# jayleicn/ClipBERT

Hardware: NVIDIA H100
Metric: clips/sec fwd+bwd MSRVTT ret (ResNet50+BERT-base) (higher is better)
Workload: dtype bf16

## Files before the change

### clipbert_b200/csrc/gemm.cu

```cuda
#include "common.cuh"
#include "host_util.h"

namespace cb {

constexpr int BM = 128;
constexpr int BK = 64;
constexpr int CONSUMER_WARPS = 8;
constexpr int GEMM_THREADS = (CONSUMER_WARPS + 1) * 32;
constexpr int PP_THREADS = 3 * 128;
constexpr int PP_PRODUCER_REGS = 40;
constexpr int PP_CONSUMER_REGS = 232;
constexpr int PP_BAR_TURN = 1;
constexpr int MAX_STAGES = 8;
constexpr int SMEM_LIMIT = 232448;
constexpr int SMEM_LIMIT_OCC2 = 113 * 1024;
constexpr int STG_PITCH = 36;
constexpr int STG_WARP_FLOATS = 16 * STG_PITCH;
constexpr int EPI_BYTES = CONSUMER_WARPS * STG_WARP_FLOATS * 4;
constexpr int IN_BOX_BYTES = BM * 64 * 2;

struct GemmEpi {
  const float* scale;
  const float* shift;
  const __nv_bfloat16* residual;
  const __nv_bfloat16* aux;
  int aux_mode;
  int act;
  void* out;
  int64_t out_ld;
  int out_fp32;
  __nv_bfloat16* out2;
  int64_t out2_ld;
  int rowmap, H, W;
  uint32_t drop_thresh;
  float drop_inv_keep;
  uint64_t seed;
  const uint64_t* seed_off;
  int mn3d;
  long long* dbg;
};

__device__ __forceinline__ void dbg_stamp(const GemmEpi& epi, int slot) {
  if (epi.dbg) {
    epi.dbg[blockIdx.x * 32 + slot] = clock64();
    if (slot == 0 || slot == 11) {
      unsigned long long ns;
      asm volatile("mov.u64 %0, %%globaltimer;" : "=l"(ns));
      epi.dbg[blockIdx.x * 32 + (slot == 0 ? 12 : 13)] = static_cast<long long>(ns);
    }
  }
}

template <int BN>
struct GemmCfg {
  static constexpr int A_BYTES = BM * BK * 2;
  static constexpr int B_BYTES = BN * BK * 2;
  static constexpr int STAGE_BYTES = A_BYTES + B_BYTES;
  static constexpr int BAR_BYTES = 256;
};

enum { EK_GENERIC = 0, EK_SHIFT_ACT = 1, EK_RELU_MASK = 2, EK_DROP_RES = 3, EK_GELU_STASH = 4, EK_AUX_MUL = 5 };

template <int NC>
__device__ __forceinline__ void add_shift(float (&f)[NC], const float (&shv)[NC]) {
#pragma unroll
  for (int j = 0; j < NC; ++j) f[j] += shv[j];
}
template <int NC>
__device__ __forceinline__ void add_residual(float (&f)[NC], const uint32_t (&res16)[NC / 2]) {
#pragma unroll
  for (int j = 0; j < NC / 2; ++j) {
    const float2 r2 = unpack_bf16x2(res16[j]);
    f[2 * j] += r2.x;
    f[2 * j + 1] += r2.y;
  }
}
template <int NC>
__device__ __forceinline__ void epilogue_shift_act(float (&f)[NC], const float (&shv)[NC], bool has_shift, const uint32_t (&res16)[NC / 2], bool has_res,
                                                   bool relu) {
  if (has_shift) add_shift<NC>(f, shv);
  if (has_res) add_residual<NC>(f, res16);
  if (relu) {
#pragma unroll
    for (int j = 0; j < NC; ++j) f[j] = fmaxf(f[j], 0.0f);
  }
}
template <int NC>
__device__ __forceinline__ void epilogue_relu_mask(float (&f)[NC], const uint32_t (&res16)[NC / 2], bool has_res, const uint32_t (&aux16)[NC / 2]) {
  if (has_res) add_residual<NC>(f, res16);
#pragma unroll
  for (int j = 0; j < NC / 2; ++j) {
    const uint32_t a = aux16[j];
    f[2 * j] = ((a & 0x8000u) == 0u && (a & 0x7fffu) != 0u) ? f[2 * j] : 0.0f;
    f[2 * j + 1] = ((a & 0x80000000u) == 0u && (a & 0x7fff0000u) != 0u) ? f[2 * j + 1] : 0.0f;
  }
}
template <int NC>
__device__ __forceinline__ void epilogue_drop_res(float (&f)[NC], const float (&shv)[NC], bool has_shift, const uint32_t (&res16)[NC / 2], bool has_res,
                                                  uint64_t dseed, uint64_t didx, uint32_t thresh, float inv_keep) {
  if (has_shift) add_shift<NC>(f, shv);
#pragma unroll
  for (int j = 0; j < NC; j += 4) {
    float m[4];
    dropout_mult4(dseed, didx + j, thresh, inv_keep, m);
    f[j] *= m[0]; f[j + 1] *= m[1]; f[j + 2] *= m[2]; f[j + 3] *= m[3];
  }
  if (has_res) add_residual<NC>(f, res16);
}
template <int NC>
__device__ __forceinline__ void epilogue_gelu_stash(float (&f)[NC], const float (&shv)[NC], bool has_shift, uint32_t (&o2_16)[NC / 2]) {
  if (has_shift) add_shift<NC>(f, shv);
#pragma unroll
  for (int j = 0; j < NC / 2; ++j) {
    float y0, g0, y1, g1;
    gelu_erf_and_grad(f[2 * j], y0, g0);
    gelu_erf_and_grad(f[2 * j + 1], y1, g1);
    f[2 * j] = y0;
    f[2 * j + 1] = y1;
    o2_16[j] = pack_bf16x2(g0, g1);
  }
}
template <int NC>
__device__ __forceinline__ void epilogue_aux_mul(float (&f)[NC], const uint32_t (&res16)[NC / 2], bool has_res, const uint32_t (&aux16)[NC / 2]) {
  if (has_res) add_residual<NC>(f, res16);
#pragma unroll
  for (int j = 0; j < NC / 2; ++j) {
    const float2 a2 = unpack_bf16x2(aux16[j]);
    f[2 * j] *= a2.x;
    f[2 * j + 1] *= a2.y;
  }
}
template <int NC, bool GUARD>
__device__ __forceinline__ void epilogue_math(float (&f)[NC], const GemmEpi& epi, const float (&shv)[NC], bool has_shift, uint64_t dseed, int nb, int N,
                                              int64_t orow, const uint32_t (&res16)[NC / 2], bool has_res, const uint32_t (&aux16)[NC / 2], bool has_aux,
                                              uint32_t (&o2_16)[NC / 2], bool has_out2) {
  if (GUARD && nb >= N) return;
  if (epi.scale) {
#pragma unroll
    for (int j = 0; j < NC; j += 4) {
      if (!GUARD || nb + j + 4 <= N) {
        const float4 s4 = __ldg(reinterpret_cast<const float4*>(epi.scale + nb + j));
        f[j] *= s4.x; f[j + 1] *= s4.y; f[j + 2] *= s4.z; f[j + 3] *= s4.w;
      }
    }
  }
  if (has_shift) add_shift<NC>(f, shv);
  if (epi.drop_thresh) {
    const uint64_t base = static_cast<uint64_t>(orow) * static_cast<uint64_t>(N) + nb;
#pragma unroll
    for (int j = 0; j < NC; j += 4) {
      float m[4];
      dropout_mult4(dseed, base + j, epi.drop_thresh, epi.drop_inv_keep, m);
      f[j] *= m[0]; f[j + 1] *= m[1]; f[j + 2] *= m[2]; f[j + 3] *= m[3];
    }
  }
  if (has_res) add_residual<NC>(f, res16);
  if (epi.act == CB_ACT_GELU_STASH_GRAD) {
#pragma unroll
    for (int j = 0; j < NC / 2; ++j) {
      float y0, g0, y1, g1;
      gelu_erf_and_grad(f[2 * j], y0, g0);
      gelu_erf_and_grad(f[2 * j + 1], y1, g1);
      f[2 * j] = y0;
      f[2 * j + 1] = y1;
      if (has_out2) o2_16[j] = pack_bf16x2(g0, g1);
    }
  } else if (has_out2) {
#pragma unroll
// ... 323 lines not shown
    while (s >= STAGES) { s -= STAGES; ph ^= 1; }
  };
  if (wg == 1) ring_skip(tile_stages);

  const int er = lane & 15, eh = lane >> 4;
  float* stg = reinterpret_cast<float*>(stg_base) + (warp - 4) * STG_WARP_FLOATS;
  const bool has_out2 = epi.out2 != nullptr;
  const bool has_shift = epi.shift != nullptr;
  const bool full = (N & 15) == 0 && epi.scale == nullptr;
  const bool drop = epi.drop_thresh != 0;
  int kind = EK_GENERIC;
  if (full) {
    if (!drop && !has_out2 && !has_aux && (epi.act == CB_ACT_NONE || epi.act == CB_ACT_RELU)) kind = EK_SHIFT_ACT;
    else if (!drop && !has_out2 && !has_shift && has_aux && epi.aux_mode == CB_AUX_RELU_MASK && epi.act == CB_ACT_NONE) kind = EK_RELU_MASK;
    else if (drop && !has_out2 && !has_aux && epi.act == CB_ACT_NONE) kind = EK_DROP_RES;
    else if (!drop && has_out2 && !has_aux && !has_res && epi.act == CB_ACT_GELU_STASH_GRAD) kind = EK_GELU_STASH;
    else if (!drop && !has_out2 && !has_shift && has_aux && epi.aux_mode == CB_AUX_MUL && epi.act == CB_ACT_NONE) kind = EK_AUX_MUL;
  }
  const bool kind_relu = epi.act == CB_ACT_RELU;
  const bool guard = (N & 15) != 0;

  for (int local = wg, tile = unit + wg * n_units; tile < total_tiles; local += 2, tile += 2 * n_units) {
    const TileInfo t = decode_tile<BN, MODE>(tile, tiles_m, tiles_n, K, ntaps, 0);
    if (local > 0) named_bar_sync(PP_BAR_TURN + wg, 2 * 128);
    const int pass = tile + n_units < total_tiles ? PP_BAR_TURN + (wg ^ 1) : 0;
    mma_tile_pp<BN, MODE != 0>(acc, smem0, stage_bytes, KCH, STAGES, n_iters, lane, s, ph, full_bar, empty_bar, pass, in_stage);

    const uint32_t in_buf = N_IN ? smem_u32(in_base) + (N_IN == 2 ? wg : 0) * in_bytes : smem0 + s * stage_bytes;
    if (in_bytes) {
      if (N_IN) mbar_wait_unguarded(&in_full[wg], static_cast<uint32_t>(local >> 1) & 1u);
      else mbar_wait_unguarded(&full_bar[s], ph);
    }
    int orow_half[2];
#pragma unroll
    for (int h = 0; h < 2; ++h) {
      const int m = t.m0 + h * 64 + wq * 16 + er;
      bool row_ok = m < M;
      int64_t orow = m;
      if (epi.rowmap == CB_ROWMAP_PAD) {
        const int hw = epi.H * epi.W;
        const int img = m / hw;
        const int r = m - img * hw;
        const int y = r / epi.W, x = r - y * epi.W;
        orow = (static_cast<int64_t>(img) * (epi.H + 2) + y + 1) * (epi.W + 2) + x + 1;
      } else if (epi.rowmap == CB_ROWMAP_UNPAD) {
        const int wp = epi.W + 2, hp = epi.H + 2;
        const int img = m / (hp * wp);
        const int r = m - img * (hp * wp);
        const int y = r / wp, x = r - y * wp;
        row_ok = row_ok && y >= 1 && y <= epi.H && x >= 1 && x <= epi.W;
        orow = (static_cast<int64_t>(img) * epi.H + (y - 1)) * epi.W + (x - 1);
      }
      orow_half[h] = row_ok ? static_cast<int>(orow) : -1;
    }
#pragma unroll
    for (int sc = 0; sc < BN / 32; ++sc) {
#pragma unroll 1
      for (int h = 0; h < 2; ++h) {
        const int wrow = h * 64 + wq * 16;
        __syncwarp();
#pragma unroll
        for (int jj = 0; jj < 4; ++jj) {
          const int j = sc * 4 + jj;
          float* p = stg + (lane >> 2) * STG_PITCH + jj * 8 + 2 * (lane & 3);
          const bool h1 = h != 0;
          *reinterpret_cast<float2*>(p) = make_float2(h1 ? acc[1][4 * j] : acc[0][4 * j], h1 ? acc[1][4 * j + 1] : acc[0][4 * j + 1]);
          *reinterpret_cast<float2*>(p + 8 * STG_PITCH) =
              make_float2(h1 ? acc[1][4 * j + 2] : acc[0][4 * j + 2], h1 ? acc[1][4 * j + 3] : acc[0][4 * j + 3]);
        }
        __syncwarp();
        const int nb = t.n0 + sc * 32 + eh * 16;
        const int64_t orow = h ? orow_half[1] : orow_half[0];
        if (orow < 0 || nb >= N) continue;
        constexpr int NC = 16;
        float f[NC];
        const uint32_t srow = smem_u32(stg + er * STG_PITCH + eh * 16);
#pragma unroll
        for (int j = 0; j < NC / 4; ++j) {
          const uint4 u = lds128(srow + j * 16);
          f[4 * j] = __uint_as_float(u.x); f[4 * j + 1] = __uint_as_float(u.y);
          f[4 * j + 2] = __uint_as_float(u.z); f[4 * j + 3] = __uint_as_float(u.w);
        }
        uint32_t res16[NC / 2], aux16[NC / 2];
        const int tc = sc * 32 + eh * 16;
        const int q = (tc & 63) >> 3;
        if (has_res) {
#pragma unroll
          for (int j = 0; j < 2; ++j) {
            const uint4 u = lds128(swz128(in_buf + (tc >> 6) * IN_BOX_BYTES, wrow + er, q + j));
            res16[4 * j] = u.x; res16[4 * j + 1] = u.y; res16[4 * j + 2] = u.z; res16[4 * j + 3] = u.w;
          }
        }
        if (has_aux) {
#pragma unroll
          for (int j = 0; j < 2; ++j) {
            const uint4 u = lds128(swz128(in_buf + (has_res ? IN_TILE_BYTES : 0) + (tc >> 6) * IN_BOX_BYTES, wrow + er, q + j));
            aux16[4 * j] = u.x; aux16[4 * j + 1] = u.y; aux16[4 * j + 2] = u.z; aux16[4 * j + 3] = u.w;
          }
        }
        float shv[NC];
        if (has_shift) {
#pragma unroll
          for (int j = 0; j < NC; j += 4) {
            float4 s4 = make_float4(0.f, 0.f, 0.f, 0.f);
            if (nb + j + 4 <= N) s4 = __ldg(reinterpret_cast<const float4*>(epi.shift + nb + j));
            shv[j] = s4.x; shv[j + 1] = s4.y; shv[j + 2] = s4.z; shv[j + 3] = s4.w;
          }
        }
        uint32_t o2_16[NC / 2];
        switch (kind) {
          case EK_SHIFT_ACT: epilogue_shift_act<NC>(f, shv, has_shift, res16, has_res, kind_relu); break;
          case EK_RELU_MASK: epilogue_relu_mask<NC>(f, res16, has_res, aux16); break;
          case EK_DROP_RES:
            epilogue_drop_res<NC>(f, shv, has_shift, res16, has_res, dseed, static_cast<uint64_t>(orow) * static_cast<uint64_t>(N) + nb,
                                  epi.drop_thresh, epi.drop_inv_keep);
            break;
          case EK_GELU_STASH: epilogue_gelu_stash<NC>(f, shv, has_shift, o2_16); break;
          case EK_AUX_MUL: epilogue_aux_mul<NC>(f, res16, has_res, aux16); break;
          default:
            if (guard) epilogue_math<NC, true>(f, epi, shv, has_shift, dseed, nb, N, orow, res16, has_res, aux16, has_aux, o2_16, has_out2);
            else epilogue_math<NC, false>(f, epi, shv, has_shift, dseed, nb, N, orow, res16, has_res, aux16, has_aux, o2_16, has_out2);
        }
        if (epi.out_fp32) {
          float* o = reinterpret_cast<float*>(epi.out) + orow * epi.out_ld + nb;
#pragma unroll
          for (int j = 0; j < NC; j += 4)
            if (nb + j + 4 <= N) *reinterpret_cast<float4*>(o + j) = make_float4(f[j], f[j + 1], f[j + 2], f[j + 3]);
        } else {
          __nv_bfloat16* o = reinterpret_cast<__nv_bfloat16*>(epi.out) + orow * epi.out_ld + nb;
#pragma unroll
          for (int j = 0; j < 2; ++j)
            if (nb + 8 * j + 8 <= N)
              *reinterpret_cast<uint4*>(o + 8 * j) = make_uint4(pack_bf16x2(f[8 * j], f[8 * j + 1]), pack_bf16x2(f[8 * j + 2], f[8 * j + 3]),
                                                                pack_bf16x2(f[8 * j + 4], f[8 * j + 5]), pack_bf16x2(f[8 * j + 6], f[8 * j + 7]));
        }
        if (has_out2) {
          __nv_bfloat16* o = epi.out2 + orow * epi.out2_ld + nb;
#pragma unroll
          for (int j = 0; j < 2; ++j)
            if (nb + 8 * j + 8 <= N) *reinterpret_cast<uint4*>(o + 8 * j) = make_uint4(o2_16[4 * j], o2_16[4 * j + 1], o2_16[4 * j + 2], o2_16[4 * j + 3]);
        }
      }
    }
    if (in_bytes) {
      __syncwarp();
      if (lane == 0) mbar_arrive(N_IN ? &in_empty[N_IN == 2 ? wg : 0] : &empty_bar[s]);
      if (!N_IN && ++s == STAGES) { s = 0; ph ^= 1; }
    }
    ring_skip(tile_stages);
  }
  if (threadIdx.x == 4 * 32) dbg_stamp(epi, 11);
}

template <int BN, int OCC>
__global__ void __launch_bounds__(GEMM_THREADS, OCC)
    gemm_kernel(const __grid_constant__ CUtensorMap tmA, const __grid_constant__ CUtensorMap tmB, int M, int N, int K, int ntaps, int tap_w,
                int tap_sign, int iters_per_split, int tiles_m, int tiles_n, int total_tiles, int STAGES, int KCH, GemmEpi epi) {
  using Cfg = GemmCfg<BN>;
  extern __shared__ uint8_t smem_raw[];
  uint8_t* smem = reinterpret_cast<uint8_t*>((reinterpret_cast<uintptr_t>(smem_raw) + 1023) & ~static_cast<uintptr_t>(1023));
  const int stage_bytes = KCH * Cfg::STAGE_BYTES;
  uint64_t* full_bar = reinterpret_cast<uint64_t*>(smem + STAGES * stage_bytes);
  uint64_t* empty_bar = full_bar + MAX_STAGES;

  const int warp = threadIdx.x >> 5;
  const int lane = threadIdx.x & 31;
  const int unit = blockIdx.x;
  const int n_units = gridDim.x;
  if (threadIdx.x == 0) dbg_stamp(epi, 0);
  pdl_trigger();
  if (threadIdx.x == 0) {
    tma_prefetch_desc(&tmA);
    tma_prefetch_desc(&tmB);
    for (int s = 0; s < STAGES; ++s) {
      mbar_init(&full_bar[s], 1);
      mbar_init(&empty_bar[s], CONSUMER_WARPS);
    }
    fence_mbar_init();
  }
  __syncthreads();
  pdl_wait();
  if (threadIdx.x == 0) dbg_stamp(epi, 1);

  if (warp >= CONSUMER_WARPS) {
    if (warp == CONSUMER_WARPS && lane == 0) {
      int s = 0;
      uint32_t ph = 0;
      for (int tile = unit; tile < total_tiles; tile += n_units) {
        const TileInfo t = decode_tile<BN, 1>(tile, tiles_m, tiles_n, K, ntaps, iters_per_split);
        int shift = 0;
        if (ntaps == 9) shift = tap_sign * ((t.tap / 3 - 1) * tap_w + (t.tap % 3 - 1));
        for (int i = 0; i < t.n_iters; i += KCH) {
          const int nch = min(KCH, t.n_iters - i);
          mbar_wait(&empty_bar[s], ph ^ 1);
          mbar_expect_tx(&full_bar[s], nch * Cfg::STAGE_BYTES);
          int kit = t.it_begin + i;
          for (int ch = 0; ch < nch; ++ch, ++kit) {
            uint8_t* sa = smem + s * stage_bytes + ch * Cfg::STAGE_BYTES;
            uint8_t* sb = sa + Cfg::A_BYTES;
            const int p = kit * BK;
            if (epi.mn3d) {
              tma_load_3d(sa, &tmA, &full_bar[s], 0, p, t.m0 >> 6);
              tma_load_3d(sb, &tmB, &full_bar[s], 0, p + shift, t.nb0 >> 6);
            } else {
#pragma unroll
              for (int j = 0; j < BM / 64; ++j) tma_load_2d(sa + j * (BK * 128), &tmA, &full_bar[s], t.m0 + j * 64, p);
#pragma unroll
              for (int j = 0; j < BN / 64; ++j) tma_load_2d(sb + j * (BK * 128), &tmB, &full_bar[s], t.nb0 + j * 64, p + shift);
            }
          }
          if (++s == STAGES) { s = 0; ph ^= 1; }
          if (i == 0 && tile == unit) dbg_stamp(epi, 2);
        }
      }
      dbg_stamp(epi, 3);
    }
    return;
  }

  const int wg = warp >> 2;
  const int wrow = wg * 64 + (warp & 3) * 16;
  const uint32_t smem0 = smem_u32(smem);
  float acc[BN / 2];
  int s = 0;
  uint32_t ph = 0;
  int local = 0;
  for (int tile = unit; tile < total_tiles; tile += n_units, ++local) {
    const TileInfo t = decode_tile<BN, 1>(tile, tiles_m, tiles_n, K, ntaps, iters_per_split);
    if (local == 0 && warp == 0 && lane == 0) dbg_stamp(epi, 4);
    mma_tile<BN, 1, 1>(acc, smem0, stage_bytes, KCH, STAGES, t.n_iters, wg, lane, s, ph, full_bar, empty_bar);
    if (local == 0 && warp == 0 && lane == 0) dbg_stamp(epi, 5);
    wgrad_epilogue<BN>(acc, reinterpret_cast<float*>(epi.out) + static_cast<int64_t>(t.tap) * N, epi.out_ld, epi.scale, M, N,
                       t.m0 + wrow + (lane >> 2), t.n0, lane);
    if (local == 0 && warp == 0 && lane == 0) dbg_stamp(epi, 8);
  }
  if (threadIdx.x == 0) dbg_stamp(epi, 11);
}

static int g_sm_limit = 0;
static int sm_count() {
  static int n = 0;
  if (n == 0) {
    int dev = 0;
    cudaGetDevice(&dev);
    cudaDeviceGetAttribute(&n, cudaDevAttrMultiProcessorCount, dev);
    if (n <= 0) n = 132;
  }
  return (g_sm_limit > 0 && g_sm_limit < n) ? g_sm_limit : n;
}

static long long* g_gemm_timeline = nullptr;
static int g_force_kch = 0;
static int g_mn3d = 1;


struct SmemPlan {
  int epi_bytes, kch, stages, chunk_bytes, n_in;
};
static SmemPlan plan_ring(int bn, bool staging, int kiters, int force_kch, int occ, int in_bytes, int n_in) {
  SmemPlan p;
  const int limit = occ == 2 ? SMEM_LIMIT_OCC2 : SMEM_LIMIT;
  p.chunk_bytes = BM * BK * 2 + bn * BK * 2;
  p.epi_bytes = staging ? EPI_BYTES : 0;
  p.n_in = n_in;
  const int chunks_fit = (limit - 1024 - GemmCfg<64>::BAR_BYTES - p.epi_bytes - n_in * in_bytes) / p.chunk_bytes;
  const int min_stages = kiters > chunks_fit ? 3 : 2;
  p.kch = 1;
  if (force_kch > 0) p.kch = force_kch;
  else if (g_force_kch > 0) p.kch = g_force_kch;
  else if (kiters >= 4 && chunks_fit >= 4 * min_stages) p.kch = 4;
  else if (kiters >= 2 && chunks_fit >= 2 * min_stages) p.kch = 2;
  if (p.kch > kiters) p.kch = kiters;
  if (p.kch > 1 && chunks_fit / p.kch < 2) p.kch = 1;
  p.stages = chunks_fit / p.kch;
  if (p.stages > MAX_STAGES) p.stages = MAX_STAGES;
  const int stage_iters = ceil_div(kiters, p.kch);
  const int cap = staging ? 2 * stage_iters + 1 : (stage_iters + 1 > 2 ? stage_iters + 1 : 2);
  if (p.stages > cap) p.stages = cap;
  return p;
}
static SmemPlan plan_smem(int bn, bool staging, int kiters, int force_kch = 0, int occ = 1, int in_bytes = 0) {
  const SmemPlan none = plan_ring(bn, staging, kiters, force_kch, occ, 0, 0);
  if (in_bytes == 0) return none;
  const SmemPlan two = plan_ring(bn, staging, kiters, force_kch, occ, in_bytes, 2);
  if (two.stages >= 2 && two.stages * two.kch >= kiters) return two;
  if (kiters > 4 && none.stages >= 2 && none.kch * none.chunk_bytes >= in_bytes) return none;
  return plan_ring(bn, staging, kiters, force_kch, occ, in_bytes, 1);
}
static int epi_in_bytes(const cb_gemm_desc& d, int bn) {
  return d.mode == CB_GEMM_WGRAD ? 0 : ((d.residual != nullptr) + (d.aux != nullptr)) * (bn / 64) * IN_BOX_BYTES;
}

template <int BN, int MODE, int OCC = 1>
static int launch_gemm(const cb_gemm_desc& d, const GemmEpi& epi_in, cudaStream_t stream) {
  static_assert(MODE == 1 || (OCC == 1 && BN <= 128), "TN / NN: one CTA per SM, 128 x 64 or 128 x 128 tiles");
  GemmEpi epi = epi_in;
  using Cfg = GemmCfg<BN>;
  constexpr int LIMIT = OCC == 2 ? SMEM_LIMIT_OCC2 : SMEM_LIMIT;
  static bool attr_set = false;
  auto kern = [] {
    if constexpr (MODE == 1) return gemm_kernel<BN, OCC>;
    else return gemm_pingpong_kernel<BN, MODE>;
  }();
  if (!attr_set) {
    cudaError_t e = cudaFuncSetAttribute(kern, cudaFuncAttributeMaxDynamicSharedMemorySize, LIMIT);
    if (e == cudaSuccess && OCC == 2)
      e = cudaFuncSetAttribute(kern, cudaFuncAttributePreferredSharedMemoryCarveout, cudaSharedmemCarveoutMaxShared);
    if (e != cudaSuccess) {
      set_error("cudaFuncSetAttribute(smem=%d): %s", LIMIT, cudaGetErrorString(e));
      return CB_ERR_CUDA;
    }
    attr_set = true;
  }
  alignas(64) CUtensorMap ta, tb, tr, tx;
  bool mn3d = false;
  int iters_per_split = 0;
  const int tiles_m = ceil_div(d.m, BM), tiles_n = ceil_div(d.n, BN);
  int total = tiles_m * tiles_n;
  int kiters;
  bool ok;
  if (MODE == 0) {
    ok = get_tmap_2d(&ta, d.a, d.k, d.a_rows, d.a_ld, BK, BM) &&
         get_tmap_2d(&tb, d.b, static_cast<uint64_t>(d.k) * d.ntaps, d.b_rows, d.b_ld, BK, BN);
    kiters = ceil_div(d.k, BK) * d.ntaps;
  } else if (MODE == 2) {
    ok = get_tmap_2d(&ta, d.a, d.k, d.a_rows, d.a_ld, BK, BM);
    mn3d = g_mn3d && d.n % 64 == 0 &&
           get_tmap_3d_mn(&tb, d.b, static_cast<uint64_t>(d.n) * d.ntaps, d.b_rows, d.b_ld, BK, BN / 64);
    if (!mn3d) ok = ok && get_tmap_2d(&tb, d.b, static_cast<uint64_t>(d.n) * d.ntaps, d.b_rows, d.b_ld, 64, BK);
    kiters = ceil_div(d.k, BK) * d.ntaps;
  } else {
    mn3d = g_mn3d && d.m % 64 == 0 && d.n % 64 == 0 && get_tmap_3d_mn(&ta, d.a, d.m, d.a_rows, d.a_ld, BK, BM / 64) &&
           get_tmap_3d_mn(&tb, d.b, d.n, d.b_rows, d.b_ld, BK, BN / 64);
    ok = mn3d || (get_tmap_2d(&ta, d.a, d.m, d.a_rows, d.a_ld, 64, BK) && get_tmap_2d(&tb, d.b, d.n, d.b_rows, d.b_ld, 64, BK));
    const int kc = ceil_div(d.k, BK);
    int splits = d.split_k < 1 ? 1 : d.split_k;
    if (splits > kc) splits = kc;
    iters_per_split = ceil_div(kc, splits);
    splits = ceil_div(kc, iters_per_split);
    total *= splits * d.ntaps;
    kiters = iters_per_split;
  }
  tr = ta;
  tx = ta;
  if (MODE != 1 && d.residual) ok = ok && get_tmap_2d(&tr, d.residual, d.n, d.m, d.res_ld, 64, BM);
  if (MODE != 1 && d.aux) ok = ok && get_tmap_2d(&tx, d.aux, d.n, d.m, d.aux_ld, 64, BM);
  if (!ok) return CB_ERR_CUDA;
  epi.mn3d = mn3d ? 1 : 0;
  const int units = sm_count() * OCC;
  const int grid = total < units ? total : units;
  const int in_bytes = epi_in_bytes(d, BN);
  const SmemPlan sp = plan_smem(BN, MODE != 1, kiters, (d.reserved >> 8) & 15, OCC, in_bytes);
  const int kch = sp.kch, stages = sp.stages;
  if (stages < 2) {
    set_error("cb_gemm: not enough shared memory for a 2-stage pipeline (BN=%d, epilogue %d B + inputs %d B, %d CTA(s) per SM)", BN,
              sp.epi_bytes, in_bytes, OCC);
    return CB_ERR_INVALID;
  }
  const int smem_bytes = stages * kch * Cfg::STAGE_BYTES + sp.n_in * in_bytes + sp.epi_bytes + Cfg::BAR_BYTES + 1024;
  if constexpr (MODE == 1)
    launch_gemm_k(kern, grid, GEMM_THREADS, smem_bytes, stream, ta, tb, d.m, d.n, d.k, d.ntaps, d.tap_w, d.tap_sign, iters_per_split,
                  tiles_m, tiles_n, total, stages, kch, epi);
  else
    launch_gemm_k(kern, grid, PP_THREADS, smem_bytes, stream, ta, tb, tr, tx, d.m, d.n, d.k, d.ntaps, d.tap_w, d.tap_sign, tiles_m,
                  tiles_n, total, stages, kch, sp.n_in, epi);
  return check_launch("cb_gemm");
}

struct LaunchCfg {
  int bn, splits;
};

static int g_occ2_mode = 1;
static double g_occ2_max_gflop = 0.0;

static LaunchCfg choose_config(const cb_gemm_desc& d, int occ = 1) {
  const int units = sm_count() * occ;
  const int kc = ceil_div(d.k, BK);
  const bool wgrad = d.mode == CB_GEMM_WGRAD;
  const int block_n = (!wgrad && d.block_n == 256) ? 128 : d.block_n;
  static const int cand[3] = {64, 128, 256};
  LaunchCfg best = {0, 1};
  double best_cost = 1e30;
  for (int c = 0; c < 3; ++c) {
    const int bn = cand[c];
    if (occ == 2 && bn > 64) continue;
    if (block_n && bn != block_n) continue;
    if (!wgrad && bn == 256) continue;
    if (bn > 64 && d.n <= bn / 2) continue;
    const int64_t base = static_cast<int64_t>(ceil_div(d.m, BM)) * ceil_div(d.n, bn) * (wgrad ? d.ntaps : 1);
    const int max_split = wgrad ? (d.split_k > 0 ? d.split_k : (kc < 32 ? kc : 32)) : 1;
    for (int sp = (wgrad && d.split_k > 0) ? d.split_k : 1; sp <= max_split; ++sp) {
      const int ips = ceil_div(wgrad ? kc : kc * d.ntaps, sp);
      const int real_sp = wgrad ? ceil_div(kc, ips) : 1;
      const int64_t tiles = base * real_sp;
      const double rounds = static_cast<double>((tiles + units - 1) / units);
      const SmemPlan pl = plan_smem(bn, !wgrad, ips, (d.reserved >> 8) & 15, occ, epi_in_bytes(d, bn));
      if (pl.stages < 2) continue;
      const double shallow = (pl.stages * pl.kch < 3 && ips > 2) ? 3.0 : 1.0;
      const double stage_cost = 450.0 + pl.kch * pl.chunk_bytes / (60.0 / occ);
      const double main_loop = ceil_div(ips, pl.kch) * stage_cost * shallow;
      double cost;
      if (wgrad) {
        cost = rounds * (main_loop + bn * 24.0) + 2500.0;
      } else {
        const double epi = bn * 30.0;
        const double per_tile = main_loop > 0.5 * (main_loop + epi) ? main_loop : 0.5 * (main_loop + epi);
        cost = rounds * per_tile + 0.5 * epi + 2500.0;
      }
      if (cost < best_cost) {
        best_cost = cost;
        best = {bn, real_sp};
      }
    }
  }
  if (best.bn == 0 && occ == 1) best = {64, 1};
  return best;
}

constexpr int WG_MAX_PROBLEMS = 8;
struct WgradProblem {
  CUtensorMap tmA, tmB;
  float* out;
  const float* scale;
  int64_t out_ld;
  int M, N, K;
  int ntaps, tap_w, tap_sign;
  int iters_per_split, tiles_m, tiles_n;
  int tile_begin;
  int mn3d;
};
struct WgradGroup {
  int nprob, total_tiles;
  WgradProblem p[WG_MAX_PROBLEMS];
};
struct WgTile {
  int pi, m0, n0, tap, it_begin, n_iters;
};
__device__ __forceinline__ WgTile wg_decode(const WgradGroup& g, int tile) {
  WgTile t;
  int pi = 0;
  while (pi + 1 < g.nprob && tile >= g.p[pi + 1].tile_begin) ++pi;
  const WgradProblem& P = g.p[pi];
  int r = tile - P.tile_begin;
  const int nt = r % P.tiles_n;
  r /= P.tiles_n;
  const int mt = r % P.tiles_m;
  r /= P.tiles_m;
  t.pi = pi;
  t.m0 = mt * BM;
  t.tap = r % P.ntaps;
  const int split = r / P.ntaps;
  const int kc = (P.K + BK - 1) / BK;
  t.it_begin = split * P.iters_per_split;
  t.n_iters = min(kc, t.it_begin + P.iters_per_split) - t.it_begin;
  t.n0 = nt;
  return t;
}

template <int BN>
__global__ void __launch_bounds__(GEMM_THREADS, 1)
    wgrad_group_kernel(const __grid_constant__ WgradGroup g, int STAGES, int KCH) {
  using Cfg = GemmCfg<BN>;
  extern __shared__ uint8_t smem_raw[];
  uint8_t* smem = reinterpret_cast<uint8_t*>((reinterpret_cast<uintptr_t>(smem_raw) + 1023) & ~static_cast<uintptr_t>(1023));
  const int stage_bytes = KCH * Cfg::STAGE_BYTES;
  uint64_t* full_bar = reinterpret_cast<uint64_t*>(smem + STAGES * stage_bytes);
  uint64_t* empty_bar = full_bar + MAX_STAGES;
  const int warp = threadIdx.x >> 5, lane = threadIdx.x & 31;
  const int unit = blockIdx.x, n_units = gridDim.x;
  pdl_trigger();
  if (threadIdx.x == 0) {
    for (int i = 0; i < g.nprob; ++i) {
      tma_prefetch_desc(&g.p[i].tmA);
      tma_prefetch_desc(&g.p[i].tmB);
    }
    for (int s = 0; s < STAGES; ++s) {
      mbar_init(&full_bar[s], 1);
      mbar_init(&empty_bar[s], CONSUMER_WARPS);
    }
    fence_mbar_init();
  }
  __syncthreads();
  pdl_wait();

  if (warp >= CONSUMER_WARPS) {
    if (warp == CONSUMER_WARPS && lane == 0) {
      int s = 0;
      uint32_t ph = 0;
      for (int tile = unit; tile < g.total_tiles; tile += n_units) {
        const WgTile t = wg_decode(g, tile);
        const WgradProblem& P = g.p[t.pi];
        const int n0 = t.n0 * BN;
        int shift = 0;
        if (P.ntaps == 9) shift = P.tap_sign * ((t.tap / 3 - 1) * P.tap_w + (t.tap % 3 - 1));
        for (int i = 0; i < t.n_iters; i += KCH) {
          const int nch = min(KCH, t.n_iters - i);
          mbar_wait(&empty_bar[s], ph ^ 1);
          mbar_expect_tx(&full_bar[s], nch * Cfg::STAGE_BYTES);
          int kit = t.it_begin + i;
          for (int ch = 0; ch < nch; ++ch, ++kit) {
            uint8_t* sa = smem + s * stage_bytes + ch * Cfg::STAGE_BYTES;
            uint8_t* sb = sa + Cfg::A_BYTES;
            const int p = kit * BK;
            if (P.mn3d) {
              tma_load_3d(sa, &P.tmA, &full_bar[s], 0, p, t.m0 >> 6);
              tma_load_3d(sb, &P.tmB, &full_bar[s], 0, p + shift, n0 >> 6);
            } else {
#pragma unroll
              for (int j = 0; j < BM / 64; ++j) tma_load_2d(sa + j * (BK * 128), &P.tmA, &full_bar[s], t.m0 + j * 64, p);
#pragma unroll
              for (int j = 0; j < BN / 64; ++j) tma_load_2d(sb + j * (BK * 128), &P.tmB, &full_bar[s], n0 + j * 64, p + shift);
            }
          }
          if (++s == STAGES) { s = 0; ph ^= 1; }
        }
      }
    }
    return;
  }

  const int wg = warp >> 2;
  const int wrow = wg * 64 + (warp & 3) * 16;
  const uint32_t smem0 = smem_u32(smem);
  float acc[BN / 2];
  int s = 0;
  uint32_t ph = 0;
  for (int tile = unit; tile < g.total_tiles; tile += n_units) {
    const WgTile t = wg_decode(g, tile);
    const WgradProblem& P = g.p[t.pi];
    mma_tile<BN, 1, 1>(acc, smem0, stage_bytes, KCH, STAGES, t.n_iters, wg, lane, s, ph, full_bar, empty_bar);
    wgrad_epilogue<BN>(acc, P.out + static_cast<int64_t>(t.tap) * P.N, P.out_ld, P.scale, P.M, P.N, t.m0 + wrow + (lane >> 2), t.n0 * BN, lane);
  }
}

template <int BN>
static int launch_wgrad_group(const cb_gemm_desc* descs, int n, int splits, cudaStream_t stream) {
  using Cfg = GemmCfg<BN>;
  static bool attr_set = false;
  auto kern = wgrad_group_kernel<BN>;
  if (!attr_set) {
    cudaError_t e = cudaFuncSetAttribute(kern, cudaFuncAttributeMaxDynamicSharedMemorySize, SMEM_LIMIT);
    if (e != cudaSuccess) {
      set_error("cudaFuncSetAttribute(smem=%d): %s", SMEM_LIMIT, cudaGetErrorString(e));
      return CB_ERR_CUDA;
    }
    attr_set = true;
  }
  alignas(64) WgradGroup g;
  g.nprob = n;
  int total = 0, max_iters = 0;
  for (int i = 0; i < n; ++i) {
    const cb_gemm_desc& d = descs[i];
    WgradProblem& P = g.p[i];
    const bool mn3d = g_mn3d && d.m % 64 == 0 && d.n % 64 == 0 && get_tmap_3d_mn(&P.tmA, d.a, d.m, d.a_rows, d.a_ld, BK, BM / 64) &&
                      get_tmap_3d_mn(&P.tmB, d.b, d.n, d.b_rows, d.b_ld, BK, BN / 64);
    if (!mn3d && !(get_tmap_2d(&P.tmA, d.a, d.m, d.a_rows, d.a_ld, 64, BK) && get_tmap_2d(&P.tmB, d.b, d.n, d.b_rows, d.b_ld, 64, BK)))
      return CB_ERR_CUDA;
    P.mn3d = mn3d ? 1 : 0;
    P.out = static_cast<float*>(d.out);
    P.scale = d.scale;
    P.out_ld = d.out_ld;
    P.M = d.m; P.N = d.n; P.K = d.k;
    P.ntaps = d.ntaps; P.tap_w = d.tap_w; P.tap_sign = d.tap_sign;
    const int kc = ceil_div(d.k, BK);
    int sp = splits < 1 ? 1 : (splits > kc ? kc : splits);
    P.iters_per_split = ceil_div(kc, sp);
    sp = ceil_div(kc, P.iters_per_split);
    P.tiles_m = ceil_div(d.m, BM);
    P.tiles_n = ceil_div(d.n, BN);
    P.tile_begin = total;
    total += P.tiles_m * P.tiles_n * d.ntaps * sp;
    if (P.iters_per_split > max_iters) max_iters = P.iters_per_split;
  }
  g.total_tiles = total;
  const SmemPlan sp = plan_smem(BN, false, max_iters, 0, 1);
  if (sp.stages < 2) {
    set_error("cb_gemm_wgrad_group: not enough shared memory for a 2-stage pipeline (BN=%d)", BN);
    return CB_ERR_INVALID;
  }
  const int smem_bytes = sp.stages * sp.kch * Cfg::STAGE_BYTES + Cfg::BAR_BYTES + 1024;
  const int units = sm_count();
  launch_gemm_k(kern, total < units ? total : units, GEMM_THREADS, smem_bytes, stream, g, sp.stages, sp.kch);
  return check_launch("cb_gemm_wgrad_group");
}

}

extern "C" void cb_debug_gemm_timeline(void* device_buf) { cb::g_gemm_timeline = static_cast<long long*>(device_buf); }
extern "C" void cb_debug_gemm_kch(int kch) { cb::g_force_kch = kch; }
extern "C" void cb_debug_gemm_mn3d(int on) { cb::g_mn3d = on ? 1 : 0; }
extern "C" void cb_debug_gemm_occ2(int mode, double max_gflop) {
  cb::g_occ2_mode = mode < 0 ? 0 : (mode > 2 ? 2 : mode);
  cb::g_occ2_max_gflop = max_gflop;
}
extern "C" void cb_debug_gemm_sm_limit(int n) { cb::g_sm_limit = n > 0 ? n : 0; }

extern "C" int cb_gemm(const cb_gemm_desc* dp, void* stream_v) {
  using namespace cb;
  CB_REQUIRE(dp != nullptr, "cb_gemm: null descriptor");
  const cb_gemm_desc& d = *dp;
  cudaStream_t stream = static_cast<cudaStream_t>(stream_v);
  CB_REQUIRE(d.a && d.b && d.out, "cb_gemm: null operand pointer");
  CB_REQUIRE(d.m > 0 && d.n > 0 && d.k > 0, "cb_gemm: empty problem m=%d n=%d k=%d", d.m, d.n, d.k);
  CB_REQUIRE(d.ntaps == 1 || d.ntaps == 9 || (d.ntaps == 4 && d.mode == CB_GEMM_TN),
             "cb_gemm: ntaps must be 1, 9 (3x3 conv) or 4 (row taps, TN only) (got %d)", d.ntaps);
  CB_REQUIRE(d.mode == CB_GEMM_TN || d.mode == CB_GEMM_WGRAD || d.mode == CB_GEMM_NN, "cb_gemm: bad mode %d", d.mode);
  CB_REQUIRE(d.dropout_p >= 0.0f && d.dropout_p < 1.0f, "cb_gemm: dropout_p out of range");

  GemmEpi epi;
  epi.scale = d.scale;
  epi.shift = d.shift;
  epi.residual = static_cast<const __nv_bfloat16*>(d.residual);
  epi.aux = static_cast<const __nv_bfloat16*>(d.aux);
  epi.aux_mode = d.aux ? d.aux_mode : CB_AUX_NONE;
  epi.act = d.act;
  epi.out = d.out;
  epi.out_ld = d.out_ld;
  epi.out_fp32 = d.out_fp32;
  epi.out2 = static_cast<__nv_bfloat16*>(d.out2);
  epi.out2_ld = d.out2_ld;
  epi.rowmap = d.rowmap;
  epi.H = d.map_h;
  epi.W = d.map_w;
  epi.seed = d.dropout_seed;
  epi.dbg = g_gemm_timeline;
  epi.mn3d = 0;
  {
    const DropCfg dc = make_drop(d.dropout_p, d.dropout_seed);
    epi.drop_thresh = dc.thresh;
    epi.drop_inv_keep = dc.inv_keep;
    epi.seed_off = dc.offset;
  }
  const double gflop = 2.0e-9 * d.m * d.n * d.k * d.ntaps;
  const bool want_occ2 = (d.reserved & 64) == 0 && (!d.block_n || d.block_n == 64) &&
                         ((d.reserved & 32) ? g_occ2_mode >= 1 : (g_occ2_mode == 2 && (g_occ2_max_gflop <= 0.0 || gflop <= g_occ2_max_gflop)));

  if (d.mode == CB_GEMM_TN || d.mode == CB_GEMM_NN) {
    const bool nn = d.mode == CB_GEMM_NN;
    CB_REQUIRE(d.n % 8 == 0, "cb_gemm(TN): n must be a multiple of 8 (got %d)", d.n);
    CB_REQUIRE(d.k % 8 == 0, "cb_gemm(TN): k must be a multiple of 8 (got %d)", d.k);
    CB_REQUIRE(d.out_ld % 8 == 0, "cb_gemm(TN): out_ld must be a multiple of 8");
    CB_REQUIRE(!d.residual || d.res_ld % 8 == 0, "cb_gemm(TN): res_ld must be a multiple of 8");
    CB_REQUIRE(!d.aux || d.aux_ld % 8 == 0, "cb_gemm(TN): aux_ld must be a multiple of 8");
    CB_REQUIRE((reinterpret_cast<uintptr_t>(d.residual) & 15) == 0, "cb_gemm(TN): residual must be 16-byte aligned");
    CB_REQUIRE((reinterpret_cast<uintptr_t>(d.aux) & 15) == 0, "cb_gemm(TN): aux must be 16-byte aligned");
    CB_REQUIRE(!d.out2 || d.out2_ld % 8 == 0, "cb_gemm(TN): out2_ld must be a multiple of 8");
    CB_REQUIRE(!(d.out2 && d.out_fp32), "cb_gemm(TN): out2 requires a bf16 primary output");
    CB_REQUIRE(d.rowmap == CB_ROWMAP_NONE || (d.map_h > 0 && d.map_w > 0), "cb_gemm: rowmap needs map_h/map_w");
    CB_REQUIRE(d.ntaps == 1 || d.tap_w > 2, "cb_gemm: tap modes need tap_w (padded row pitch in pixels)");
    CB_REQUIRE(d.block_n == 0 || d.block_n == 64 || d.block_n == 128 || d.block_n == 256, "cb_gemm: block_n must be 0, 64, 128 or 256 (got %d)",
               d.block_n);
    const LaunchCfg lc = choose_config(d);
    switch (lc.bn) {
      case 64: return nn ? launch_gemm<64, 2>(d, epi, stream) : launch_gemm<64, 0>(d, epi, stream);
      case 128: return nn ? launch_gemm<128, 2>(d, epi, stream) : launch_gemm<128, 0>(d, epi, stream);
      default: CB_REQUIRE(false, "cb_gemm: no tile width for block_n %d", d.block_n);
    }
  } else {
    CB_REQUIRE(d.out_fp32 == 1, "cb_gemm(WGRAD): output must be fp32");
    CB_REQUIRE(d.m % 8 == 0 && d.n % 8 == 0, "cb_gemm(WGRAD): m, n must be multiples of 8 (got %d, %d)", d.m, d.n);
    CB_REQUIRE(d.out_ld % 4 == 0, "cb_gemm(WGRAD): out_ld must be a multiple of 4");
    CB_REQUIRE((reinterpret_cast<uintptr_t>(d.out) & 15) == 0, "cb_gemm(WGRAD): out must be 16-byte aligned");
    if (want_occ2) {
      const LaunchCfg l2 = choose_config(d, 2);
      cb_gemm_desc d2 = d;
      d2.split_k = l2.splits;
      if (l2.bn == 64) return launch_gemm<64, 1, 2>(d2, epi, stream);
    }
    const LaunchCfg lc = choose_config(d);
    cb_gemm_desc d2 = d;
    d2.split_k = lc.splits;
    switch (lc.bn) {
      case 64: return launch_gemm<64, 1>(d2, epi, stream);
      case 128: return launch_gemm<128, 1>(d2, epi, stream);
      case 256: return launch_gemm<256, 1>(d2, epi, stream);
      default: CB_REQUIRE(false, "cb_gemm(WGRAD): block_n must be 0, 64, 128 or 256 (got %d)", lc.bn);
    }
  }
  return CB_ERR_INVALID;
}

extern "C" int cb_gemm_wgrad_group(const cb_gemm_desc* descs, int n, void* stream_v) {
  using namespace cb;
  CB_REQUIRE(descs != nullptr && n >= 1, "cb_gemm_wgrad_group: no problems");
  cudaStream_t stream = static_cast<cudaStream_t>(stream_v);
  bool groupable = n >= 2 && n <= WG_MAX_PROBLEMS;
  for (int i = 0; i < n; ++i) {
    const cb_gemm_desc& d = descs[i];
    CB_REQUIRE(d.mode == CB_GEMM_WGRAD && d.out_fp32 == 1, "cb_gemm_wgrad_group: problem %d is not an fp32 WGRAD descriptor", i);
    CB_REQUIRE(d.a && d.b && d.out && d.m > 0 && d.n > 0 && d.k > 0, "cb_gemm_wgrad_group: problem %d: null operand / empty shape", i);
    CB_REQUIRE(d.m % 8 == 0 && d.n % 8 == 0 && d.out_ld % 4 == 0 && (reinterpret_cast<uintptr_t>(d.out) & 15) == 0,
               "cb_gemm_wgrad_group: problem %d: m, n multiples of 8, out 16-byte aligned, out_ld a multiple of 4", i);
    CB_REQUIRE(d.ntaps == 1 || d.ntaps == 9, "cb_gemm_wgrad_group: problem %d: ntaps must be 1 or 9", i);
    if (d.k * 2 < descs[0].k || descs[0].k * 2 < d.k) groupable = false;
  }
  if (!groupable) {
    for (int i = 0; i < n; ++i) {
      const int rc = cb_gemm(&descs[i], stream_v);
      if (rc != CB_OK) return rc;
    }
    return CB_OK;
  }
  int min_n = descs[0].n;
  for (int i = 1; i < n; ++i) min_n = descs[i].n < min_n ? descs[i].n : min_n;
  const int bn = min_n >= 192 ? 256 : (min_n >= 96 ? 128 : 64);
  int64_t base = 0;
  int kc_min = 1 << 30;
  for (int i = 0; i < n; ++i) {
    base += static_cast<int64_t>(ceil_div(descs[i].m, BM)) * ceil_div(descs[i].n, bn) * descs[i].ntaps;
    const int kc = ceil_div(descs[i].k, BK);
    kc_min = kc < kc_min ? kc : kc_min;
  }
  const int sms = sm_count();
  int best_split = 1;
  double best_cost = 1e30;
  for (int sp = 1; sp <= 8 && sp <= kc_min; ++sp) {
    const double waves = static_cast<double>((base * sp + sms - 1) / sms);
    const double cost = waves / sp + 0.06 * sp;
    if (cost < best_cost) { best_cost = cost; best_split = sp; }
  }
  if (bn == 256) return launch_wgrad_group<256>(descs, n, best_split, stream);
  if (bn == 128) return launch_wgrad_group<128>(descs, n, best_split, stream);
  return launch_wgrad_group<64>(descs, n, best_split, stream);
}
```

Before: 3809.

## Drop two-CTA-per-SM WGRAD path and retune grouped split-K cost model

Removes the occupancy-2 WGRAD GEMM variant, so all weight-gradient GEMMs run one CTA per SM with the full shared-memory budget. The grouped WGRAD split-K choice now uses a cost model of waves times per-split K iterations plus a fixed overhead, and honours block_n and split_k overrides from the descriptor. Warp index is also made warp-uniform via a shuffle so the compiler can treat role branches as uniform. The risk is losing the occupancy-2 latency hiding on small GEMMs, and the new split heuristic may pick different splits.

```diff
diff --git a/clipbert_b200/csrc/gemm.cu b/clipbert_b200/csrc/gemm.cu
--- a/clipbert_b200/csrc/gemm.cu
+++ b/clipbert_b200/csrc/gemm.cu
@@ -13,7 +13,6 @@
 constexpr int PP_BAR_TURN = 1;
 constexpr int MAX_STAGES = 8;
 constexpr int SMEM_LIMIT = 232448;
-constexpr int SMEM_LIMIT_OCC2 = 113 * 1024;
 constexpr int STG_PITCH = 36;
 constexpr int STG_WARP_FLOATS = 16 * STG_PITCH;
 constexpr int EPI_BYTES = CONSUMER_WARPS * STG_WARP_FLOATS * 4;
@@ -643,8 +642,8 @@
   if (threadIdx.x == 4 * 32) dbg_stamp(epi, 11);
 }
 
-template <int BN, int OCC>
-__global__ void __launch_bounds__(GEMM_THREADS, OCC)
+template <int BN>
+__global__ void __launch_bounds__(GEMM_THREADS, 1)
     gemm_kernel(const __grid_constant__ CUtensorMap tmA, const __grid_constant__ CUtensorMap tmB, int M, int N, int K, int ntaps, int tap_w,
                 int tap_sign, int iters_per_split, int tiles_m, int tiles_n, int total_tiles, int STAGES, int KCH, GemmEpi epi) {
   using Cfg = GemmCfg<BN>;
@@ -654,7 +653,7 @@
   uint64_t* full_bar = reinterpret_cast<uint64_t*>(smem + STAGES * stage_bytes);
   uint64_t* empty_bar = full_bar + MAX_STAGES;
 
-  const int warp = threadIdx.x >> 5;
+  const int warp = __shfl_sync(0xffffffffu, static_cast<int>(threadIdx.x >> 5), 0);
   const int lane = threadIdx.x & 31;
   const int unit = blockIdx.x;
   const int n_units = gridDim.x;
@@ -748,9 +747,9 @@
 struct SmemPlan {
   int epi_bytes, kch, stages, chunk_bytes, n_in;
 };
-static SmemPlan plan_ring(int bn, bool staging, int kiters, int force_kch, int occ, int in_bytes, int n_in) {
+static SmemPlan plan_ring(int bn, bool staging, int kiters, int force_kch, int in_bytes, int n_in) {
   SmemPlan p;
-  const int limit = occ == 2 ? SMEM_LIMIT_OCC2 : SMEM_LIMIT;
+  const int limit = SMEM_LIMIT;
   p.chunk_bytes = BM * BK * 2 + bn * BK * 2;
   p.epi_bytes = staging ? EPI_BYTES : 0;
   p.n_in = n_in;
@@ -770,35 +769,32 @@
   if (p.stages > cap) p.stages = cap;
   return p;
 }
-static SmemPlan plan_smem(int bn, bool staging, int kiters, int force_kch = 0, int occ = 1, int in_bytes = 0) {
-  const SmemPlan none = plan_ring(bn, staging, kiters, force_kch, occ, 0, 0);
+static SmemPlan plan_smem(int bn, bool staging, int kiters, int force_kch = 0, int in_bytes = 0) {
+  const SmemPlan none = plan_ring(bn, staging, kiters, force_kch, 0, 0);
   if (in_bytes == 0) return none;
-  const SmemPlan two = plan_ring(bn, staging, kiters, force_kch, occ, in_bytes, 2);
+  const SmemPlan two = plan_ring(bn, staging, kiters, force_kch, in_bytes, 2);
   if (two.stages >= 2 && two.stages * two.kch >= kiters) return two;
   if (kiters > 4 && none.stages >= 2 && none.kch * none.chunk_bytes >= in_bytes) return none;
-  return plan_ring(bn, staging, kiters, force_kch, occ, in_bytes, 1);
+  return plan_ring(bn, staging, kiters, force_kch, in_bytes, 1);
 }
 static int epi_in_bytes(const cb_gemm_desc& d, int bn) {
   return d.mode == CB_GEMM_WGRAD ? 0 : ((d.residual != nullptr) + (d.aux != nullptr)) * (bn / 64) * IN_BOX_BYTES;
 }
 
-template <int BN, int MODE, int OCC = 1>
+template <int BN, int MODE>
 static int launch_gemm(const cb_gemm_desc& d, const GemmEpi& epi_in, cudaStream_t stream) {
-  static_assert(MODE == 1 || (OCC == 1 && BN <= 128), "TN / NN: one CTA per SM, 128 x 64 or 128 x 128 tiles");
+  static_assert(MODE == 1 || BN <= 128, "TN / NN: 128 x 64 or 128 x 128 tiles");
   GemmEpi epi = epi_in;
   using Cfg = GemmCfg<BN>;
-  constexpr int LIMIT = OCC == 2 ? SMEM_LIMIT_OCC2 : SMEM_LIMIT;
   static bool attr_set = false;
   auto kern = [] {
-    if constexpr (MODE == 1) return gemm_kernel<BN, OCC>;
+    if constexpr (MODE == 1) return gemm_kernel<BN>;
     else return gemm_pingpong_kernel<BN, MODE>;
   }();
   if (!attr_set) {
-    cudaError_t e = cudaFuncSetAttribute(kern, cudaFuncAttributeMaxDynamicSharedMemorySize, LIMIT);
-    if (e == cudaSuccess && OCC == 2)
-      e = cudaFuncSetAttribute(kern, cudaFuncAttributePreferredSharedMemoryCarveout, cudaSharedmemCarveoutMaxShared);
+    cudaError_t e = cudaFuncSetAttribute(kern, cudaFuncAttributeMaxDynamicSharedMemorySize, SMEM_LIMIT);
     if (e != cudaSuccess) {
-      set_error("cudaFuncSetAttribute(smem=%d): %s", LIMIT, cudaGetErrorString(e));
+      set_error("cudaFuncSetAttribute(smem=%d): %s", SMEM_LIMIT, cudaGetErrorString(e));
       return CB_ERR_CUDA;
     }
     attr_set = true;
@@ -838,14 +834,14 @@
   if (MODE != 1 && d.aux) ok = ok && get_tmap_2d(&tx, d.aux, d.n, d.m, d.aux_ld, 64, BM);
   if (!ok) return CB_ERR_CUDA;
   epi.mn3d = mn3d ? 1 : 0;
-  const int units = sm_count() * OCC;
+  const int units = sm_count();
   const int grid = total < units ? total : units;
   const int in_bytes = epi_in_bytes(d, BN);
-  const SmemPlan sp = plan_smem(BN, MODE != 1, kiters, (d.reserved >> 8) & 15, OCC, in_bytes);
+  const SmemPlan sp = plan_smem(BN, MODE != 1, kiters, (d.reserved >> 8) & 15, in_bytes);
   const int kch = sp.kch, stages = sp.stages;
   if (stages < 2) {
-    set_error("cb_gemm: not enough shared memory for a 2-stage pipeline (BN=%d, epilogue %d B + inputs %d B, %d CTA(s) per SM)", BN,
-              sp.epi_bytes, in_bytes, OCC);
+    set_error("cb_gemm: not enough shared memory for a 2-stage pipeline (BN=%d, epilogue %d B + inputs %d B)", BN, sp.epi_bytes,
+              in_bytes);
     return CB_ERR_INVALID;
   }
   const int smem_bytes = stages * kch * Cfg::STAGE_BYTES + sp.n_in * in_bytes + sp.epi_bytes + Cfg::BAR_BYTES + 1024;
@@ -862,20 +858,16 @@
   int bn, splits;
 };
 
-static int g_occ2_mode = 1;
-static double g_occ2_max_gflop = 0.0;
-
-static LaunchCfg choose_config(const cb_gemm_desc& d, int occ = 1) {
-  const int units = sm_count() * occ;
+static LaunchCfg choose_config(const cb_gemm_desc& d) {
+  const int units = sm_count();
   const int kc = ceil_div(d.k, BK);
   const bool wgrad = d.mode == CB_GEMM_WGRAD;
   const int block_n = (!wgrad && d.block_n == 256) ? 128 : d.block_n;
   static const int cand[3] = {64, 128, 256};
-  LaunchCfg best = {0, 1};
+  LaunchCfg best = {64, 1};
   double best_cost = 1e30;
   for (int c = 0; c < 3; ++c) {
     const int bn = cand[c];
-    if (occ == 2 && bn > 64) continue;
     if (block_n && bn != block_n) continue;
     if (!wgrad && bn == 256) continue;
     if (bn > 64 && d.n <= bn / 2) continue;
@@ -886,10 +878,10 @@
       const int real_sp = wgrad ? ceil_div(kc, ips) : 1;
       const int64_t tiles = base * real_sp;
       const double rounds = static_cast<double>((tiles + units - 1) / units);
-      const SmemPlan pl = plan_smem(bn, !wgrad, ips, (d.reserved >> 8) & 15, occ, epi_in_bytes(d, bn));
+      const SmemPlan pl = plan_smem(bn, !wgrad, ips, (d.reserved >> 8) & 15, epi_in_bytes(d, bn));
       if (pl.stages < 2) continue;
       const double shallow = (pl.stages * pl.kch < 3 && ips > 2) ? 3.0 : 1.0;
-      const double stage_cost = 450.0 + pl.kch * pl.chunk_bytes / (60.0 / occ);
+      const double stage_cost = 450.0 + pl.kch * pl.chunk_bytes / 60.0;
       const double main_loop = ceil_div(ips, pl.kch) * stage_cost * shallow;
       double cost;
       if (wgrad) {
@@ -905,7 +897,6 @@
       }
     }
   }
-  if (best.bn == 0 && occ == 1) best = {64, 1};
   return best;
 }
 
@@ -958,7 +949,8 @@
   const int stage_bytes = KCH * Cfg::STAGE_BYTES;
   uint64_t* full_bar = reinterpret_cast<uint64_t*>(smem + STAGES * stage_bytes);
   uint64_t* empty_bar = full_bar + MAX_STAGES;
-  const int warp = threadIdx.x >> 5, lane = threadIdx.x & 31;
+  const int warp = __shfl_sync(0xffffffffu, static_cast<int>(threadIdx.x >> 5), 0);
+  const int lane = threadIdx.x & 31;
   const int unit = blockIdx.x, n_units = gridDim.x;
   pdl_trigger();
   if (threadIdx.x == 0) {
@@ -1065,7 +1057,7 @@
     if (P.iters_per_split > max_iters) max_iters = P.iters_per_split;
   }
   g.total_tiles = total;
-  const SmemPlan sp = plan_smem(BN, false, max_iters, 0, 1);
+  const SmemPlan sp = plan_smem(BN, false, max_iters);
   if (sp.stages < 2) {
     set_error("cb_gemm_wgrad_group: not enough shared memory for a 2-stage pipeline (BN=%d)", BN);
     return CB_ERR_INVALID;
@@ -1081,10 +1073,7 @@
 extern "C" void cb_debug_gemm_timeline(void* device_buf) { cb::g_gemm_timeline = static_cast<long long*>(device_buf); }
 extern "C" void cb_debug_gemm_kch(int kch) { cb::g_force_kch = kch; }
 extern "C" void cb_debug_gemm_mn3d(int on) { cb::g_mn3d = on ? 1 : 0; }
-extern "C" void cb_debug_gemm_occ2(int mode, double max_gflop) {
-  cb::g_occ2_mode = mode < 0 ? 0 : (mode > 2 ? 2 : mode);
-  cb::g_occ2_max_gflop = max_gflop;
-}
+extern "C" void cb_debug_gemm_occ2(int, double) {}
 extern "C" void cb_debug_gemm_sm_limit(int n) { cb::g_sm_limit = n > 0 ? n : 0; }
 
 extern "C" int cb_gemm(const cb_gemm_desc* dp, void* stream_v) {
@@ -1123,9 +1112,6 @@
     epi.drop_inv_keep = dc.inv_keep;
     epi.seed_off = dc.offset;
   }
-  const double gflop = 2.0e-9 * d.m * d.n * d.k * d.ntaps;
-  const bool want_occ2 = (d.reserved & 64) == 0 && (!d.block_n || d.block_n == 64) &&
-                         ((d.reserved & 32) ? g_occ2_mode >= 1 : (g_occ2_mode == 2 && (g_occ2_max_gflop <= 0.0 || gflop <= g_occ2_max_gflop)));
 
   if (d.mode == CB_GEMM_TN || d.mode == CB_GEMM_NN) {
     const bool nn = d.mode == CB_GEMM_NN;
@@ -1153,12 +1139,6 @@
     CB_REQUIRE(d.m % 8 == 0 && d.n % 8 == 0, "cb_gemm(WGRAD): m, n must be multiples of 8 (got %d, %d)", d.m, d.n);
     CB_REQUIRE(d.out_ld % 4 == 0, "cb_gemm(WGRAD): out_ld must be a multiple of 4");
     CB_REQUIRE((reinterpret_cast<uintptr_t>(d.out) & 15) == 0, "cb_gemm(WGRAD): out must be 16-byte aligned");
-    if (want_occ2) {
-      const LaunchCfg l2 = choose_config(d, 2);
-      cb_gemm_desc d2 = d;
-      d2.split_k = l2.splits;
-      if (l2.bn == 64) return launch_gemm<64, 1, 2>(d2, epi, stream);
-    }
     const LaunchCfg lc = choose_config(d);
     cb_gemm_desc d2 = d;
     d2.split_k = lc.splits;
@@ -1193,24 +1173,28 @@
     }
     return CB_OK;
   }
+  CB_REQUIRE(descs[0].block_n == 0 || descs[0].block_n == 64 || descs[0].block_n == 128 || descs[0].block_n == 256,
+             "cb_gemm_wgrad_group: block_n must be 0, 64, 128 or 256 (got %d)", descs[0].block_n);
   int min_n = descs[0].n;
   for (int i = 1; i < n; ++i) min_n = descs[i].n < min_n ? descs[i].n : min_n;
-  const int bn = min_n >= 192 ? 256 : (min_n >= 96 ? 128 : 64);
+  const int bn = descs[0].block_n ? descs[0].block_n : (min_n >= 192 ? 256 : (min_n >= 96 ? 128 : 64));
   int64_t base = 0;
-  int kc_min = 1 << 30;
+  int kc_min = 1 << 30, kc_max = 0;
   for (int i = 0; i < n; ++i) {
     base += static_cast<int64_t>(ceil_div(descs[i].m, BM)) * ceil_div(descs[i].n, bn) * descs[i].ntaps;
     const int kc = ceil_div(descs[i].k, BK);
     kc_min = kc < kc_min ? kc : kc_min;
+    kc_max = kc > kc_max ? kc : kc_max;
   }
   const int sms = sm_count();
   int best_split = 1;
   double best_cost = 1e30;
   for (int sp = 1; sp <= 8 && sp <= kc_min; ++sp) {
     const double waves = static_cast<double>((base * sp + sms - 1) / sms);
-    const double cost = waves / sp + 0.06 * sp;
+    const double cost = waves * (ceil_div(kc_max, sp) + 8.0);
     if (cost < best_cost) { best_cost = cost; best_split = sp; }
   }
+  if (descs[0].split_k > 0) best_split = descs[0].split_k;
   if (bn == 256) return launch_wgrad_group<256>(descs, n, best_split, stream);
   if (bn == 128) return launch_wgrad_group<128>(descs, n, best_split, stream);
   return launch_wgrad_group<64>(descs, n, best_split, stream);
```

New measurement: 3983 (median of 6 runs). +4.6%, better.
